# linhthi/BLISS-GNN

Measured on AMD Instinct MI355X. Metric: steps/sec (train step: sample_blocks + gather + SAGE fwd/bwd + Adam + exp3), reddit-like, higher is better.
Workload: dtype bf16

## Files before the change

bliss_gnn_amd/_engine.py:

```python
import contextlib
import ctypes as C
import os

import numpy as np
import torch

from . import _lib
from .graph import Block, Graph

_CHUNK = 1024
_CAP_ERRS = 1 | 2 | 4 | 8 | 64


def _ptr(t):
    return 0 if t is None else t.data_ptr()


def _stream():
    return torch.cuda.current_stream().cuda_stream


def _up8(n):
    return (int(n) + 7) & ~7


class _LayerWs:

    def __init__(self, dev, cap_s, cap_c):
        self.cap_s, self.cap_c = cap_s, cap_c
        self.seg_ptr = torch.empty(cap_s + 1, dtype=torch.int32, device=dev)
        self.seed_acc = torch.empty(60 * cap_s + 64, dtype=torch.uint8, device=dev)
        self.cand_nid = torch.empty(cap_c, dtype=torch.int32, device=dev)
        self.new_id = torch.empty(cap_c, dtype=torch.int32, device=dev)
        self.p = torch.empty(cap_c, dtype=torch.bfloat16, device=dev)
        self.P = torch.empty(cap_c, dtype=torch.bfloat16, device=dev)
        self.uniforms = torch.empty(cap_c, dtype=torch.float32, device=dev)
        self.keys = torch.empty(cap_c, dtype=torch.float32, device=dev)
        self.draw_scr = torch.zeros(int(_lib.lib.bliss_multinomial_draw_scratch_bytes(cap_c)) // 4, dtype=torch.int32, device=dev)
        self.src_cnt = None
        self.tr_temp = None


class DrawState:

    def __init__(self, seed, step, device):
        self.seed = int(seed) & ((1 << 64) - 1)
        self.step_dev = torch.tensor([int(step)], dtype=torch.int64, device=device)

    def step(self):
        return int(self.step_dev.item())


class LayerEngine:

    def __init__(self, g: Graph):
        if g.device.type != "cuda":
            raise RuntimeError("bliss_gnn_amd samples on the GPU only; move the graph with g.to('cuda') "
                               "(the reference's --data-cpu/--use-uva modes are out of scope)")
        self.g = g
        dev = g.device
        V = g.num_nodes()
        self.V, self.Eg = V, g.num_edges()
        if self.Eg >= 2 ** 31:
            raise RuntimeError("int32 edge positions: graphs with >= 2^31 edges are not supported")
        self.scratch_sets = 2
        self._sets = {}
        self.first_pos = torch.full((V,), -1, dtype=torch.int32, device=dev)
        self.acc_p2 = torch.zeros(V, dtype=torch.int64, device=dev)
        self.c_graph = _lib.Graph(g.indptr.data_ptr(), g.indices.data_ptr(), _ptr(g.eid), V, self.Eg)
        self.flags = torch.zeros(16, dtype=torch.int32, device=dev)
        self.fs_ticket = torch.zeros(1, dtype=torch.int32, device=dev)
        self.fuse_scale = os.environ.get("BLISS_FUSE_SCALE", "1") != "0"
        self.flag_err = torch.zeros(1, dtype=torch.int32, device=dev)
        self.n_bins = 0
        for nb in ((int(os.environ["BLISS_NBINS"]),) if os.environ.get("BLISS_NBINS") else (256, 1024)):
            if -(-V // nb) * 12 <= 64 * 1024:
                self.n_bins = nb
                break
        if os.environ.get("BLISS_BINS", "1") == "0" or self.Eg > 2048 * 4096 * 32:
            self.n_bins = 0
        self._bins = None
        self.hist = torch.zeros(32768, dtype=torch.int32, device=dev)
        self.mt_dev = torch.empty(626, dtype=torch.int32, device=dev)
        self.mt_host = torch.empty(626, dtype=torch.int32).pin_memory()
# ... 714 lines not shown
```

bliss_gnn_amd/csrc/common.cuh:

```cuda
#pragma once
#include <hip/hip_runtime.h>
#include <stdint.h>
#include "bliss_gnn.h"

#define BLISS_WAVE 64

#define FRAC_DST 40
#define FRAC_SRC 44
#define FRAC_BLK 36

#define BLISS_ERR_CAP_FRONTIER 1
#define BLISS_ERR_CAP_CAND     2
#define BLISS_ERR_CAP_KEPT     4
#define BLISS_ERR_CAP_EDGES    8
#define BLISS_ERR_NONFINITE   16
#define BLISS_ERR_FIXED_RANGE 32
#define BLISS_ERR_CAP_SEEDS   64
#define BLISS_ERR_RNG_STREAM 128
#define BLISS_ERR_FLAG_TIMEOUT 256

typedef uint16_t bf16_t;

__device__ __forceinline__ float bf2f(bf16_t b) { return __uint_as_float(((uint32_t)b) << 16); }

// ... 52 lines not shown

__device__ __forceinline__ long long bf_to_fixed_wide(bf16_t b, int frac, long long* lo, int* sticky, int* bad) {
  uint32_t e = (b >> 7) & 0xff, m = b & 0x7f;
  if (e == 255) { *bad |= BLISS_ERR_NONFINITE; return 0; }
  if (e == 0) e = 1; else m |= 0x80;
  const int shift = (int)e - 134 + frac;
  const bool neg = (b & 0x8000) != 0;
  if (shift >= 0) {
    if (shift > 55) { *bad |= BLISS_ERR_FIXED_RANGE; return 0; }
    const long long mag = (long long)((uint64_t)m << shift);
    return neg ? -mag : mag;
  }
  const int rs = -shift;
  const uint32_t top = rs >= 8 ? 0u : (m >> rs);
  const uint32_t r = rs >= 8 ? m : (m & ((1u << rs) - 1u));
  if (r) {
    long long l;
    if (rs <= 40) l = (long long)((uint64_t)r << (40 - rs));
    else {
      const int d = rs - 40;
      l = d >= 8 ? 0 : (long long)(r >> d);
      if (d >= 8 || (r & ((1u << d) - 1u))) *sticky = 1;
    }
    *lo += neg ? -l : l;
  }
  return neg ? -(long long)top : (long long)top;
}

__device__ __forceinline__ bf16_t fixed_wide_to_bf(int64_t hi, int64_t lo, int sticky, int frac, int* bad) {
  if (lo == 0 && !sticky) return fixed_to_bf(hi, frac, bad);
  __int128 t = ((__int128)hi << 40) + (__int128)lo;
  if (t == 0) return 0;
  const uint32_t sign = t < 0 ? 0x8000u : 0u;
  const unsigned __int128 mag = t < 0 ? (unsigned __int128)(-t) : (unsigned __int128)t;
  const uint64_t mh = (uint64_t)(mag >> 64), ml = (uint64_t)mag;
  const int msb = mh ? 127 - __clzll((long long)mh) : 63 - __clzll((long long)ml);
  const int f = frac + 40;
  auto round_shift = [&](int sh) -> uint64_t {
    if (sh <= 0) return (uint64_t)(mag << (-sh));
    if (sh > 126) return 0;
    uint64_t q = (uint64_t)(mag >> sh);
    const unsigned __int128 rem = mag & ((((unsigned __int128)1) << sh) - 1), half = ((unsigned __int128)1) << (sh - 1);
    if (rem > half || (rem == half && (sticky || (q & 1)))) q += 1;
    return q;
  };
  if (msb - f + 127 <= 0) return (bf16_t)(sign | (uint32_t)round_shift(f - 133));
  uint64_t q = round_shift(msb - 7);
  int e = msb - f + 127;
  if (q >= 256) { q >>= 1; e += 1; }
  if (e >= 255) { *bad |= BLISS_ERR_FIXED_RANGE; return 0; }
  return (bf16_t)(sign | ((uint32_t)e << 7) | ((uint32_t)q & 0x7f));
}

__device__ __forceinline__ int lane_id() { return threadIdx.x & (BLISS_WAVE - 1); }

__device__ __forceinline__ int64_t shfl_up_i64(int64_t v, int d) {
  int lo = __shfl_up((int)(v & 0xffffffffll), d), hi = __shfl_up((int)(v >> 32), d);
  return ((int64_t)hi << 32) | (uint32_t)lo;
}

template <int CTRL, int ROW_MASK>
__device__ __forceinline__ int dpp_mov0(int v) { return __builtin_amdgcn_update_dpp(0, v, CTRL, ROW_MASK, 0xf, false); }
template <int CTRL, int ROW_MASK>
__device__ __forceinline__ long long dpp_mov0_i64(long long v) {
  const int lo = dpp_mov0<CTRL, ROW_MASK>((int)(v & 0xffffffffll)), hi = dpp_mov0<CTRL, ROW_MASK>((int)(v >> 32));
  return ((long long)hi << 32) | (unsigned)lo;
}
__device__ __forceinline__ int wave_total_i32(int v) {
  v += dpp_mov0<0x111, 0xf>(v); v += dpp_mov0<0x112, 0xf>(v); v += dpp_mov0<0x114, 0xf>(v); v += dpp_mov0<0x118, 0xf>(v);
  v += dpp_mov0<0x142, 0xa>(v); v += dpp_mov0<0x143, 0xc>(v);
  return __builtin_amdgcn_readlane(v, 63);
}
__device__ __forceinline__ int wave_max_u31(int v) {
  v = max(v, dpp_mov0<0x111, 0xf>(v)); v = max(v, dpp_mov0<0x112, 0xf>(v)); v = max(v, dpp_mov0<0x114, 0xf>(v));
  v = max(v, dpp_mov0<0x118, 0xf>(v)); v = max(v, dpp_mov0<0x142, 0xa>(v)); v = max(v, dpp_mov0<0x143, 0xc>(v));
  return __builtin_amdgcn_readlane(v, 63);
}
__device__ __forceinline__ int bf_exp_field(bf16_t b) { const int e = (b >> 7) & 0xff; return e == 0 ? 1 : e; }
__device__ __forceinline__ int rel_frac(int frac, int emax) { const int s = 126 - emax; return frac + (s > 0 ? s : 0); }

__device__ __forceinline__ long long wave_total_i64(long long v) {
  v += dpp_mov0_i64<0x111, 0xf>(v); v += dpp_mov0_i64<0x112, 0xf>(v); v += dpp_mov0_i64<0x114, 0xf>(v);
  v += dpp_mov0_i64<0x118, 0xf>(v); v += dpp_mov0_i64<0x142, 0xa>(v); v += dpp_mov0_i64<0x143, 0xc>(v);
  const int lo = __builtin_amdgcn_readlane((int)(v & 0xffffffffll), 63), hi = __builtin_amdgcn_readlane((int)(v >> 32), 63);
  return ((long long)hi << 32) | (unsigned)lo;
}
__device__ __forceinline__ bool wave_single_key(int key, int* k0) {
  const unsigned long long act = __ballot(key >= 0);
  if (!act) { *k0 = -1; return true; }
  *k0 = __builtin_amdgcn_readlane(key, __ffsll((long long)act) - 1);
  return __ballot(key >= 0 && key != *k0) == 0ull;
}

__device__ __forceinline__ void wave_segsum_atomic_i64(int key, int64_t v, unsigned long long* acc) {
  const int lane = lane_id();
  int k0;
  if (wave_single_key(key, &k0)) {
    if (k0 < 0) return;
    const long long tot = wave_total_i64(key >= 0 ? v : 0);
    if (lane == 0 && tot != 0) atomicAdd(acc + k0, (unsigned long long)tot);
    return;
  }
#pragma unroll
  for (int d = 1; d < BLISS_WAVE; d <<= 1) {
    int64_t vu = shfl_up_i64(v, d);
    int ku = __shfl_up(key, d);
// ... 117 lines not shown
```

bliss_gnn_amd/csrc/sampler.hip:

```cpp
#include "common.cuh"
#include "bliss_gnn.h"
#include "prof.h"
#include "edge_q.cuh"
#include <cstdlib>

#ifndef TPB
#define TPB 256
#endif
#define ITEMS 4
#define CHUNK (TPB * ITEMS)

namespace {

#define SPAN (64 * ITEMS)
#define SEG_ZERO_WGS 8
#define LONG_COL 1024

struct EdgeAt {
  int k;
  int64_t pos;
  int src;
};

__device__ __forceinline__ EdgeAt decode(int base, int E, int S, const int* __restrict__ seg_ptr,
                                         const long long* __restrict__ col_base, const int* __restrict__ indices, int* k_hint) {
  EdgeAt r;
  const int e = base + lane_id();
  r.k = wave_segment(seg_ptr, S, base, k_hint);
  r.pos = 0; r.src = 0;
  if (e < E) {
    r.pos = col_base[r.k] + e;
    r.src = indices[r.pos];
  } else r.k = -1;
  return r;
}

__device__ __forceinline__ int chunk_wave_offset(int wave_total, int* sh4, int* chunk_total) {
  const int wave = threadIdx.x >> 6;
  __syncthreads();
  if (lane_id() == 0) sh4[wave] = wave_total;
  __syncthreads();
  int off = 0, tot = 0;
#pragma unroll
  for (int w = 0; w < TPB / 64; ++w) { const int v = sh4[w]; tot += v; if (w < wave) off += v; }
  *chunk_total = tot;
  return off;
}

__device__ __forceinline__ void seg_scan_body(const int64_t* __restrict__ indptr, const int* __restrict__ seeds,
                                              LayerCounts* cnt, int S_host, const int* __restrict__ S_dev, int cap_s,
                                              unsigned long long* __restrict__ seed_acc, int* __restrict__ seg_ptr,
                                              int* __restrict__ local_id, int num_nodes, int* __restrict__ src_cnt, int cap_k,
                                              int* __restrict__ bin_cursor, int n_bins, long long* __restrict__ col_base,
                                              int* __restrict__ span_seg, long long frontier_cap, int* entry_flag,
                                              int wg, int n_wgs, bool keep_sums, int* sh, int* st_sh, int* hub_count = nullptr) {
  if (entry_flag && wg == 0 && threadIdx.x == 0) __hip_atomic_store(entry_flag, 1, __ATOMIC_RELEASE, __HIP_MEMORY_SCOPE_AGENT);
  __shared__ int sh_long;
  if (hub_count && threadIdx.x == 0) sh_long = 0;
  int S = S_host >= 0 ? S_host : *S_dev;
  int bad = 0;
  if (S > cap_s) { S = cap_s; bad |= BLISS_ERR_CAP_SEEDS; }
  if (wg > 0 || n_wgs == 1) {
    const int nz = n_wgs > 1 ? n_wgs - 1 : 1, bz = n_wgs > 1 ? wg - 1 : 0;
    const int t0 = bz * blockDim.x + threadIdx.x, step = nz * blockDim.x;
    for (int i = (keep_sums ? 2 * cap_s : 0) + t0; i < cap_s * 5; i += step) seed_acc[i] = 0ull;
    if (src_cnt) for (int i = t0; i <= cap_k; i += step) src_cnt[i] = 0;
    if (bin_cursor) for (int i = t0; i <= n_bins; i += step) bin_cursor[i] = 0;
    for (int k = t0; k < S; k += step) { const int s = seeds[k]; if (s >= 0 && s < num_nodes) local_id[s] = k; }
    if (n_wgs > 1) return;
  }
  long long run = 0;
  constexpr int G = 4;
  for (int base0 = 0; base0 < S; base0 += G * (int)blockDim.x) {
    int degs[G];
    long long cols[G];
#pragma unroll
    for (int i = 0; i < G; ++i) {
      const int k = base0 + i * (int)blockDim.x + threadIdx.x;
      degs[i] = 0; cols[i] = 0;
      if (k < S) {
        const int s = seeds[k];
        if (s < 0 || s >= num_nodes) { bad |= BLISS_ERR_CAP_CAND; }
        else {
          cols[i] = indptr[s];
          degs[i] = (int)(indptr[s + 1] - cols[i]);
        }
      }
    }
#pragma unroll
    for (int i = 0; i < G; ++i) {
      const int k = base0 + i * (int)blockDim.x + threadIdx.x;
      if (base0 + i * (int)blockDim.x >= S) break;
      const int deg = degs[i];
      int tot, ex = block_excl_scan(deg, sh, &tot);
      const long long start = run + ex;
      if (k < S) {
        seg_ptr[k] = (int)start;
        col_base[k] = deg > 0 ? cols[i] - start : 0;
      }
      if (hub_count) {
        const bool is_long = k < S && deg > LONG_COL;
        const unsigned long long mask = __ballot(is_long);
        if (mask) {
          int base_l = 0;
          if (lane_id() == 0) base_l = atomicAdd(&sh_long, __popcll(mask));
          base_l = __shfl(base_l, 0);
          if (is_long) hub_count[base_l + __popcll(mask & ((1ull << lane_id()) - 1ull))] = k;
        }
      }
      if (run + tot <= frontier_cap) {
        st_sh[threadIdx.x] = (int)(k < S ? start : run + tot);
        __syncthreads();
        const long long sp_end = (run + tot + SPAN - 1) / SPAN;
        for (long long sp = (run + SPAN - 1) / SPAN + threadIdx.x; sp < sp_end; sp += blockDim.x) {
          const int p = (int)(sp * SPAN);
          int t = 0;
#pragma unroll
          for (int step = 512; step >= 1; step >>= 1) if (st_sh[t + step] <= p) t += step;
          span_seg[sp] = base0 + i * (int)blockDim.x + t;
        }
      }
      run += tot;
      if (run > frontier_cap) bad |= BLISS_ERR_CAP_FRONTIER;
    }
  }
  int any_bad = __syncthreads_or(bad);
  if (threadIdx.x == 0) {
    if (hub_count) hub_count[cap_s] = sh_long;
    seg_ptr[S] = (int)run;
    cnt->S = S; cnt->E = (any_bad & BLISS_ERR_CAP_FRONTIER) ? 0 : (int)run;
    cnt->C = 0; cnt->K = 0; cnt->B = 0; cnt->iters = 0; cnt->all_one = 0; cnt->c = 1.0;
    cnt->err = any_bad;
  }
}

__global__ void __launch_bounds__(1024) k_seg_scan(const int64_t* __restrict__ indptr, const int* __restrict__ seeds,
                                                   LayerCounts* cnt, int S_host, const int* __restrict__ S_dev, int cap_s,
                                                   unsigned long long* __restrict__ seed_acc, int* __restrict__ seg_ptr,
                                                   int* __restrict__ local_id, int num_nodes, int* __restrict__ src_cnt, int cap_k,
                                                   int* __restrict__ bin_cursor, int n_bins, long long* __restrict__ col_base,
                                                   int* __restrict__ span_seg, long long frontier_cap, int* entry_flag,
                                                   int keep_sums, int* hub_count) {
  __shared__ int sh[17];
  __shared__ int st_sh[1024];
  seg_scan_body(indptr, seeds, cnt, S_host, S_dev, cap_s, seed_acc, seg_ptr, local_id, num_nodes, src_cnt, cap_k, bin_cursor, n_bins,
                col_base, span_seg, frontier_cap, entry_flag, blockIdx.x, gridDim.x, keep_sums != 0, sh, st_sh, hub_count);
}

template <bool BANDIT>
__global__ void __launch_bounds__(TPB) k_frontier_pass1(const int64_t* __restrict__ indptr, const int* __restrict__ indices,
                                                        const bf16_t* __restrict__ w, const int* __restrict__ seeds,
                                                        const int* __restrict__ seg_ptr, const long long* __restrict__ col_base,
    const int* __restrict__ span_seg, LayerCounts* cnt,
                                                        const int* __restrict__ local_id, unsigned* first_pos,
                                                        unsigned long long* acc_w) {
  const int S = cnt->S, E = cnt->E;
  const int nspans = (E + SPAN - 1) / SPAN;
  int bad = 0;
  for (int sp = blockIdx.x * (TPB / 64) + (threadIdx.x >> 6); sp < nspans; sp += gridDim.x * (TPB / 64)) {
    int hint = span_seg[sp];
#pragma unroll
    for (int i = 0; i < ITEMS; ++i) {
      const int base = sp * SPAN + i * 64;
      if (base >= E) break;
      const int e = base + lane_id();
      EdgeAt a = decode(base, E, S, seg_ptr, col_base, indices, &hint);
      int64_t term = 0;
      if (a.k >= 0) {
        if (local_id[a.src] < 0) {
          if (__hip_atomic_load(first_pos + a.src, __ATOMIC_RELAXED, __HIP_MEMORY_SCOPE_AGENT) > (unsigned)e)
            atomicMin(first_pos + a.src, (unsigned)e);
        }
        if (BANDIT) term = bf_to_fixed(w[a.pos], FRAC_DST, &bad);
      }
      if (BANDIT) wave_segsum_atomic_i64(a.k, term, acc_w);
    }
  }
  if (bad) atomicOr(&cnt->err, bad);
}

template <bool BANDIT>
__global__ void __launch_bounds__(TPB) k_frontier_pass2(const int64_t* __restrict__ indptr, const int* __restrict__ indices,
                                                        const bf16_t* __restrict__ w, const int* __restrict__ seeds,
                                                        const int* __restrict__ seg_ptr, const long long* __restrict__ col_base,
    const int* __restrict__ span_seg, LayerCounts* cnt,
                                                        const unsigned* __restrict__ first_pos,
                                                        const unsigned long long* __restrict__ acc_w,
                                                        unsigned long long* acc_q, int* __restrict__ chunk_cnt,
                                                        float eta_f, float ome_f) {
  __shared__ int sh4[TPB / 64];
  const int S = cnt->S, E = cnt->E;
  const int nchunks = (E + CHUNK - 1) / CHUNK;
  int bad = 0;
  for (int chunk = blockIdx.x; chunk < nchunks; chunk += gridDim.x) {
    int nfirst = 0, hint = span_seg[chunk * ITEMS + (threadIdx.x >> 6)];
#pragma unroll
    for (int i = 0; i < ITEMS; ++i) {
      const int base = chunk * CHUNK + (threadIdx.x >> 6) * SPAN + i * 64;
      if (base >= E) break;
// ... 114 lines not shown
  __shared__ int lh[HIST_BINS];
  const int S = cnt->S;
  const int C = min(cnt->C, cap_c);
  if ((int)blockIdx.x * FIN_TPB >= C) return;
  {
    int4* lh4 = reinterpret_cast<int4*>(lh);
    for (int b = threadIdx.x; b < HIST_BINS / 4; b += FIN_TPB) lh4[b] = make_int4(0, 0, 0, 0);
  }
  __syncthreads();
  int bad = 0;
  for (int id = blockIdx.x * FIN_TPB + threadIdx.x; id < C; id += gridDim.x * FIN_TPB) {
    int g;
    if (id < S) { g = seeds[id]; cand_nid[id] = g; } else g = cand_nid[id];
    const unsigned long long raw = acc_p2[g];
    acc_p2[g] = 0;
    first_pos[g] = 0xffffffffu;
    bf16_t pj;
    if (uniform_nodes) pj = raw ? (bf16_t)0x3f80 : (bf16_t)0;
    else pj = f2bf(sqrtf(bf2f(fixed_to_bf((int64_t)raw, FRAC_SRC, &bad))));
    p[id] = pj;
    if (pj < HIST_BINS) atomicAdd(&lh[pj], 1); else bad |= BLISS_ERR_NONFINITE;
  }
  __syncthreads();
  {
    const int4* lh4 = reinterpret_cast<const int4*>(lh);
    for (int b = threadIdx.x; b < HIST_BINS / 4; b += FIN_TPB) {
      const int4 v = lh4[b];
      if (v.x | v.y | v.z | v.w) {
        if (v.x) atomicAdd(hist + 4 * b, v.x);
        if (v.y) atomicAdd(hist + 4 * b + 1, v.y);
        if (v.z) atomicAdd(hist + 4 * b + 2, v.z);
        if (v.w) atomicAdd(hist + 4 * b + 3, v.w);
      }
    }
  }
  if (bad) atomicOr(&cnt->err, bad);
}

#define BIN_TPB 1024
#ifndef BIN_ITEMS
#define BIN_ITEMS 4
#endif
#define BIN_BATCH (BIN_TPB * BIN_ITEMS)
#define MAX_BINS 1024
#ifndef COL_TPB
#define COL_TPB 1024
#endif
#ifndef COL_R
#define COL_R 16
#endif
#ifndef COL_RB
#define COL_RB 8
#endif
#define COL_BIG (COL_R * 64)
static_assert(LONG_COL == COL_BIG, "k_seg_scan lists the columns k_col_sums treats as long");
#ifndef BINRED_TPB
#define BINRED_TPB 1024
#endif

template <int NT>
__device__ __forceinline__ int block_max_u31(int v, long long* sh) {
  v = wave_max_u31(v);
  __syncthreads();
  if (lane_id() == 0) sh[threadIdx.x >> 6] = v;
  __syncthreads();
  int t = 0;
#pragma unroll
  for (int w = 0; w < NT / 64; ++w) t = max(t, (int)sh[w]);
  return t;
}

template <int NT>
__device__ __forceinline__ long long block_sum2_i64(long long a, long long b, long long* sh2, long long* b_out) {
  a = wave_total_i64(a);
  b = wave_total_i64(b);
  __syncthreads();
  if (lane_id() == 0) { sh2[threadIdx.x >> 6] = a; sh2[NT / 64 + (threadIdx.x >> 6)] = b; }
  __syncthreads();
  long long ta = 0, tb = 0;
#pragma unroll
  for (int w = 0; w < NT / 64; ++w) { ta += sh2[w]; tb += sh2[NT / 64 + w]; }
  *b_out = tb;
  return ta;
}

template <int NT>
__device__ __forceinline__ long long block_sum_i64(long long v, long long* sh) {
  v = wave_total_i64(v);
  __syncthreads();
  if (lane_id() == 0) sh[threadIdx.x >> 6] = v;
  __syncthreads();
  long long t = 0;
#pragma unroll
  for (int w = 0; w < NT / 64; ++w) t += sh[w];
  return t;
}

__device__ __forceinline__ void col_store(int k, long long ws_fixed, long long qs_fixed, bf16_t wsum, int n, float eta_f,
                                          unsigned long long* acc_w, unsigned long long* acc_q, uint2* seed_coef, int* bad) {
  acc_w[k] = (unsigned long long)ws_fixed; acc_q[k] = (unsigned long long)qs_fixed;
  const bf16_t qsum = fixed_to_bf(qs_fixed, FRAC_DST, bad);
  seed_coef[k] = make_uint2((unsigned)wsum | ((unsigned)qsum << 16), __float_as_uint(rbf((1.0f / (float)n) * eta_f)));
}

__global__ void __launch_bounds__(COL_TPB) k_col_sums(const int64_t* __restrict__ indptr, const bf16_t* __restrict__ w,
                                                      const int* __restrict__ seeds, const int* __restrict__ seg_ptr,
                                                      const long long* __restrict__ col_base, const int* __restrict__ span_seg,
                                                      LayerCounts* cnt, unsigned long long* __restrict__ acc_w,
                                                      unsigned long long* __restrict__ acc_q, float eta_f, float ome_f,
                                                      uint2* __restrict__ seed_coef, int n_wave_wgs,
                                                      const int* __restrict__ long_list, int cap_s) {
  __shared__ long long sh[COL_TPB / 64];
  __shared__ long long sh2[2 * COL_TPB / 64];
  const int S = cnt->S, tid = threadIdx.x, lane = lane_id();
  if (cnt->E == 0) return;
  int bad = 0;
  const int n_block_wgs = (int)gridDim.x - n_wave_wgs;
  if ((int)blockIdx.x < n_wave_wgs)
  for (int k = blockIdx.x * (COL_TPB / 64) + (tid >> 6); k < S; k += n_wave_wgs * (COL_TPB / 64)) {
    const int s0 = seg_ptr[k], n = seg_ptr[k + 1] - s0;
    if (n == 0 || n > COL_BIG) continue;
    const long long p0 = col_base[k] + s0;
    bf16_t wr[COL_R];
    long long part = 0;
    int emax = 1;
#pragma unroll
    for (int r = 0; r < COL_R; ++r) {
      const int i = lane + r * 64;
      wr[r] = 0;
      if (i < n) wr[r] = w[p0 + i];
    }
#pragma unroll
    for (int r = 0; r < COL_R; ++r)
      if (lane + r * 64 < n) emax = max(emax, bf_exp_field(wr[r]));
    const int wfrac = rel_frac(FRAC_DST, wave_max_u31(emax));
    long long part_lo = 0;
    int sticky = 0;
#pragma unroll
    for (int r = 0; r < COL_R; ++r)
      if (lane + r * 64 < n) part += bf_to_fixed_wide(wr[r], wfrac, &part_lo, &sticky, &bad);
    const long long ws_fixed = wave_total_i64(part);
    bf16_t wsum;
    if (__ballot(part_lo != 0 || sticky) == 0ull) wsum = fixed_to_bf(ws_fixed, wfrac, &bad);
    else wsum = fixed_wide_to_bf(ws_fixed, wave_total_i64(part_lo), __ballot(sticky) != 0ull, wfrac, &bad);
    const float a = rbf((1.0f / (float)n) * eta_f);
    part = 0;
#pragma unroll
    for (int r = 0; r < COL_R; ++r) {
      const int i = lane + r * 64;
      if (i < n) part += bf_to_fixed(edge_q_pre(wr[r], wsum, a, ome_f), FRAC_DST, &bad);
    }
    const long long qs_fixed = wave_total_i64(part);
    if (lane == 0) col_store(k, ws_fixed, qs_fixed, wsum, n, eta_f, acc_w, acc_q, seed_coef, &bad);
  }
  if ((int)blockIdx.x >= n_wave_wgs)
  for (int li = (int)blockIdx.x - n_wave_wgs, n_long = long_list[cap_s]; li < n_long; li += n_block_wgs) {
    const int k = long_list[li];
    const int s0 = seg_ptr[k], n = seg_ptr[k + 1] - s0;
    if (n <= COL_BIG) continue;
    const long long p0 = col_base[k] + s0;
    bf16_t wr[COL_RB];
    long long part = 0;
    int emax = 1;
#pragma unroll
    for (int r = 0; r < COL_RB; ++r) {
      const int i = tid + r * COL_TPB;
      wr[r] = 0;
      if (i < n) wr[r] = w[p0 + i];
    }
#pragma unroll
    for (int r = 0; r < COL_RB; ++r)
      if (tid + r * COL_TPB < n) emax = max(emax, bf_exp_field(wr[r]));
#pragma unroll 8
    for (int i = tid + COL_RB * COL_TPB; i < n; i += COL_TPB) emax = max(emax, bf_exp_field(w[p0 + i]));
    const int wfrac = rel_frac(FRAC_DST, block_max_u31<COL_TPB>(emax, sh));
    long long part_lo = 0;
    int sticky = 0;
#pragma unroll
    for (int r = 0; r < COL_RB; ++r)
      if (tid + r * COL_TPB < n) part += bf_to_fixed_wide(wr[r], wfrac, &part_lo, &sticky, &bad);
#pragma unroll 8
    for (int i = tid + COL_RB * COL_TPB; i < n; i += COL_TPB)
      part += bf_to_fixed_wide(w[p0 + i], wfrac, &part_lo, &sticky, &bad);
    long long lost;
    const long long ws_fixed = block_sum2_i64<COL_TPB>(part, (part_lo != 0 || sticky) ? 1 : 0, sh2, &lost);
    bf16_t wsum;
    if (lost == 0) wsum = fixed_to_bf(ws_fixed, wfrac, &bad);
    else {
      const long long lo_tot = block_sum_i64<COL_TPB>(part_lo, sh);
      const long long st_tot = block_sum_i64<COL_TPB>(sticky, sh);
      wsum = fixed_wide_to_bf(ws_fixed, lo_tot, st_tot != 0, wfrac, &bad);
    }
    const float a = rbf((1.0f / (float)n) * eta_f);
    part = 0;
#pragma unroll
    for (int r = 0; r < COL_RB; ++r) {
      const int i = tid + r * COL_TPB;
      if (i < n) part += bf_to_fixed(edge_q_pre(wr[r], wsum, a, ome_f), FRAC_DST, &bad);
    }
#pragma unroll 8
    for (int i = tid + COL_RB * COL_TPB; i < n; i += COL_TPB) part += bf_to_fixed(edge_q_pre(w[p0 + i], wsum, a, ome_f), FRAC_DST, &bad);
    const long long qs_fixed = block_sum_i64<COL_TPB>(part, sh);
    if (tid == 0) col_store(k, ws_fixed, qs_fixed, wsum, n, eta_f, acc_w, acc_q, seed_coef, &bad);
  }
  if (bad) atomicOr(&cnt->err, bad);
}

template <bool BANDIT>
__global__ void __launch_bounds__(BIN_TPB) k_bin_scatter(const int64_t* __restrict__ indptr, const int* __restrict__ indices,
                                                     const bf16_t* __restrict__ w, const int* __restrict__ seeds,
                                                     const int* __restrict__ seg_ptr, const long long* __restrict__ col_base,
    const int* __restrict__ span_seg, LayerCounts* cnt,
                                                     const unsigned long long* __restrict__ acc_w,
                                                     const unsigned long long* __restrict__ acc_q, float eta_f, float ome_f,
                                                     int uniform_nodes, int n_bins, int log2_bins, long long bin_cap, int* bin_cursor,
                                                     unsigned long long* __restrict__ bin_rec, unsigned* __restrict__ bitmap,
                                                     const uint2* __restrict__ seed_coef) {
  __shared__ int hist[MAX_BINS];
  __shared__ int gbase[MAX_BINS];
  const int S = cnt->S, E = cnt->E, tid = threadIdx.x;
  const int nb = (E + BIN_BATCH - 1) / BIN_BATCH;
  const int bmask = n_bins - 1;
  int bad = 0;
  for (int batch = blockIdx.x; batch < nb; batch += gridDim.x) {
    for (int b = tid; b < n_bins; b += BIN_TPB) hist[b] = 0;
    if (tid < BIN_BATCH / 32) bitmap[batch * (BIN_BATCH / 32) + tid] = 0u;
    __syncthreads();
    int srcs[BIN_ITEMS], ranks[BIN_ITEMS];
    bf16_t ts[BIN_ITEMS];
    const int wbase = batch * BIN_BATCH + (tid >> 6) * (64 * BIN_ITEMS);
    int hint = span_seg[wbase >> 8];
#pragma unroll
    for (int j = 0; j < BIN_ITEMS; ++j) {
      ranks[j] = -1; srcs[j] = 0; ts[j] = 0;
      const int base = wbase + j * 64;
      if (base >= E) continue;
      EdgeAt a = decode(base, E, S, seg_ptr, col_base, indices, &hint);
      if (a.k >= 0) {
        bf16_t t;
        if (uniform_nodes) {
          t = (bf16_t)0x3f80;
        } else if (BANDIT) {
          const uint2 cf = seed_coef[a.k];
          bf16_t q = edge_q_pre(w[a.pos], (bf16_t)(cf.x & 0xffffu), __uint_as_float(cf.y), ome_f);
          float r = rbf(bf2f(q) / bf2f((bf16_t)(cf.x >> 16)));
          t = f2bf(r * r);
        } else {
          float x = bf2f(w[a.pos]);
          t = f2bf(x * x);
        }
        srcs[j] = a.src; ts[j] = t;
        ranks[j] = atomicAdd(&hist[a.src & bmask], 1);
      }
    }
    __syncthreads();
    for (int b = tid; b < n_bins; b += BIN_TPB) {
// ... 687 lines not shown

extern "C" {

int bliss_layer_counts_bytes(void) { return (int)sizeof(LayerCounts); }

int bliss_flag_raise(int32_t* flag, void* stream) {
  if (!flag) return BLISS_EINVAL;
  k_flag_raise<<<1, 64, 0, (hipStream_t)stream>>>(flag);
  return (int)hipGetLastError();
}

int bliss_flag_wait(int32_t* flag, int32_t* err_word, void* stream) {
  if (!flag) return BLISS_EINVAL;
  k_flag_wait<<<1, 64, 0, (hipStream_t)stream>>>(flag, err_word, g_flag_spin_bound);
  return (int)hipGetLastError();
}

int bliss_flag_set_spin_bound(int64_t spins) {
  if (spins < 1) return BLISS_EINVAL;
  g_flag_spin_bound = spins;
  return 0;
}

int bliss_frontier_prob(const bliss_graph_t* g, const bliss_node_maps_t* m, const void* w_pos, const int32_t* seeds,
                        int32_t n_seeds, const int32_t* n_seeds_dev, int32_t cap_s, int mode, float eta_f,
                        float one_minus_eta_f, int64_t frontier_bound, const bliss_layer_ws_t* ws, void* stream_) {
  if (!g || !m || !seeds || !ws || !w_pos || cap_s <= 0 || !ws->hist || !ws->span_seg) return BLISS_EINVAL;
  if (n_seeds < 0 && !n_seeds_dev) return BLISS_EINVAL;
  if (n_seeds > cap_s) return BLISS_EINVAL;
  const int uniform_nodes = (mode & BLISS_MODE_UNIFORM_NODES) ? 1 : 0;
  const bool partials_only = (mode & BLISS_MODE_PARTIALS) != 0;
  mode &= ~(BLISS_MODE_UNIFORM_NODES | BLISS_MODE_PARTIALS);
  if (mode != BLISS_MODE_BANDIT && mode != BLISS_MODE_LADIES) return BLISS_EINVAL;
  if (partials_only && ws->n_bins <= 0) return BLISS_EINVAL;
  hipStream_t st = (hipStream_t)stream_;
  LayerCounts* cnt = (LayerCounts*)ws->counts;
  const bf16_t* w = (const bf16_t*)w_pos;
  unsigned long long* acc_w = (unsigned long long*)ws->seed_acc;
  unsigned long long* acc_q = acc_w + cap_s;
  const long long* col_base = (const long long*)(acc_w + 5 * (size_t)cap_s);
  if (frontier_bound < 1) frontier_bound = 1;
  const int ge = grid_for(frontier_bound, TPB), gc = grid_for(frontier_bound, CHUNK);
  const bool binned = ws->n_bins > 0;
  int log2_bins = 0, slots = 0;
  if (binned) {
    while ((1 << log2_bins) < ws->n_bins) ++log2_bins;
    slots = (g->num_nodes + ws->n_bins - 1) >> log2_bins;
    if ((1 << log2_bins) != ws->n_bins || ws->n_bins > MAX_BINS || (size_t)slots * 12 > 64 * 1024 || ws->bin_cap <= 0 ||
        g->num_edges > (long long)MAX_TILES * BTILE * 32 || !ws->bin_cursor || !ws->bin_rec || !ws->bitmap || !ws->word_prefix || !ws->touched_key || !ws->touched_sum)
      return BLISS_EINVAL;
  }
  const long long fcap = (long long)(g->num_edges < 0x7fffffffll ? g->num_edges : 0x7fffffffll);
  const bool col_sums = binned && mode == BLISS_MODE_BANDIT;
  int* long_list = (int*)(acc_w + 7 * (size_t)cap_s);
  PROF_LAUNCH(BK_SEG_SCAN, st, k_seg_scan<<<1 + SEG_ZERO_WGS, 1024, 0, st>>>(g->indptr, seeds, cnt, n_seeds, n_seeds_dev, cap_s, acc_w, ws->seg_ptr,
                                                            m->local_id, g->num_nodes, ws->src_cnt, ws->cap_k,
                                                            binned ? ws->bin_cursor : nullptr, ws->n_bins, (long long*)col_base, ws->span_seg,
                                                            fcap, ws->entry_flag, col_sums ? 1 : 0, col_sums ? long_list : nullptr));
  if (binned) {
    unsigned long long* seed_p2 = acc_w + 4 * (size_t)cap_s;
    uint2* seed_coef = (uint2*)(acc_w + 6 * (size_t)cap_s);
    unsigned long long* bin_rec = (unsigned long long*)ws->bin_rec;
    const int gb = grid_for(frontier_bound, BIN_BATCH);
    const int n_wave_wgs = grid_for(cap_s, COL_TPB / 64, 2048);
    if (col_sums)
      PROF_LAUNCH(BK_COL_SUMS, st, k_col_sums<<<n_wave_wgs + (cap_s < 2048 ? cap_s : 2048), COL_TPB, 0, st>>>(g->indptr, w, seeds, ws->seg_ptr, col_base, ws->span_seg, cnt, acc_w, acc_q, eta_f, one_minus_eta_f, seed_coef, n_wave_wgs, long_list, cap_s));
    if (mode == BLISS_MODE_BANDIT)
      PROF_LAUNCH(BK_BIN_SCATTER, st, k_bin_scatter<true><<<gb, BIN_TPB, 0, st>>>(g->indptr, g->indices, w, seeds, ws->seg_ptr, col_base, ws->span_seg, cnt, acc_w, acc_q, eta_f, one_minus_eta_f, uniform_nodes, ws->n_bins, log2_bins, ws->bin_cap, ws->bin_cursor, bin_rec, ws->bitmap, seed_coef));
    else
      PROF_LAUNCH(BK_BIN_SCATTER, st, k_bin_scatter<false><<<gb, BIN_TPB, 0, st>>>(g->indptr, g->indices, w, seeds, ws->seg_ptr, col_base, ws->span_seg, cnt, acc_w, acc_q, eta_f, one_minus_eta_f, uniform_nodes, ws->n_bins, log2_bins, ws->bin_cap, ws->bin_cursor, bin_rec, ws->bitmap, seed_coef));
    PROF_LAUNCH(BK_BIN_REDUCE, st, k_bin_reduce<<<ws->n_bins, BINRED_TPB, (size_t)slots * 12, st>>>(
        cnt, ws->n_bins, log2_bins, ws->bin_cap, ws->bin_cursor, bin_rec, g->num_nodes, slots, m->local_id, seed_p2,
        (unsigned long long*)ws->touched_key, (unsigned long long*)ws->touched_sum, ws->bitmap, ws->cap_c));
    if (partials_only) return (int)hipGetLastError();
    int* tile_sum = ws->word_prefix;
    int* word_prefix = ws->word_prefix + MAX_TILES;
    PROF_LAUNCH(BK_BITMAP_SCAN, st, k_bitmap_tiles<<<grid_for(frontier_bound, (int64_t)BTILE * 32, MAX_TILES), 1024, 0, st>>>(ws->bitmap, word_prefix, tile_sum, cnt));
    int gf = (ws->cap_c + FIN_TPB - 1) / FIN_TPB;
    if (gf < 1) gf = 1;
    if (gf > 512) gf = 512;
    PROF_LAUNCH(BK_CAND_NUMBER, st, k_cand_number<<<gf, FIN_TPB, 0, st>>>(
        seeds, cnt, ws->cand_nid, m->local_id, seed_p2, (const unsigned long long*)ws->touched_key,
        (const unsigned long long*)ws->touched_sum, ws->bitmap, word_prefix, tile_sum, (bf16_t*)ws->p, ws->hist, ws->cap_c, uniform_nodes,
        FusedScale{ws->fs_ticket, ws->fs_fanout, ws->fs_eps, ws->fs_rng_ctl, ws->fs_layer_off, ws->fs_is_last, ws->fs_rng_cap, ws->chunk_cnt}));
    return (int)hipGetLastError();
  }
  if (mode == BLISS_MODE_BANDIT) {
    PROF_LAUNCH(BK_PASS1, st, k_frontier_pass1<true><<<ge, TPB, 0, st>>>(g->indptr, g->indices, w, seeds, ws->seg_ptr, col_base, ws->span_seg, cnt, m->local_id, m->first_pos, acc_w));
    PROF_LAUNCH(BK_PASS2, st, k_frontier_pass2<true><<<gc, TPB, 0, st>>>(g->indptr, g->indices, w, seeds, ws->seg_ptr, col_base, ws->span_seg, cnt, m->first_pos, acc_w, acc_q, ws->chunk_cnt, eta_f, one_minus_eta_f));
  } else {
    PROF_LAUNCH(BK_PASS1, st, k_frontier_pass1<false><<<ge, TPB, 0, st>>>(g->indptr, g->indices, w, seeds, ws->seg_ptr, col_base, ws->span_seg, cnt, m->local_id, m->first_pos, acc_w));
    PROF_LAUNCH(BK_PASS2, st, k_frontier_pass2<false><<<gc, TPB, 0, st>>>(g->indptr, g->indices, w, seeds, ws->seg_ptr, col_base, ws->span_seg, cnt, m->first_pos, acc_w, acc_q, ws->chunk_cnt, eta_f, one_minus_eta_f));
  }
  PROF_LAUNCH(BK_CHUNK_SCAN, st, k_chunk_scan<<<1, 1024, 0, st>>>(ws->chunk_cnt, cnt, 0, ws->cap_c));
  if (mode == BLISS_MODE_BANDIT)
    PROF_LAUNCH(BK_PASS3, st, k_frontier_pass3<true><<<gc, TPB, 0, st>>>(g->indptr, g->indices, w, seeds, ws->seg_ptr, col_base, ws->span_seg, cnt, m->first_pos, acc_w, acc_q, ws->chunk_cnt, m->local_id, ws->cand_nid, (unsigned long long*)m->acc_p2, eta_f, one_minus_eta_f, ws->cap_c, uniform_nodes));
  else
    PROF_LAUNCH(BK_PASS3, st, k_frontier_pass3<false><<<gc, TPB, 0, st>>>(g->indptr, g->indices, w, seeds, ws->seg_ptr, col_base, ws->span_seg, cnt, m->first_pos, acc_w, acc_q, ws->chunk_cnt, m->local_id, ws->cand_nid, (unsigned long long*)m->acc_p2, eta_f, one_minus_eta_f, ws->cap_c, uniform_nodes));
  {
    int gf = (ws->cap_c + FIN_TPB * 8 - 1) / (FIN_TPB * 8);
    if (gf < 1) gf = 1;
    if (gf > 256) gf = 256;
    PROF_LAUNCH(BK_CAND_FINALIZE, st, k_cand_finalize<<<gf, FIN_TPB, 0, st>>>(
        seeds, cnt, ws->cand_nid, (unsigned long long*)m->acc_p2, m->first_pos, (bf16_t*)ws->p, ws->hist, ws->cap_c, uniform_nodes));
  }
  return (int)hipGetLastError();
}

int bliss_poisson_select(const bliss_layer_ws_t* ws, int32_t fanout, double eps, const float* uniforms,
                         int32_t* uniforms_offset_dev, int32_t* rng_ctl, int is_last, int32_t rng_cap_total,
                         int64_t cand_bound, void* stream_) {
  if (!ws || !uniforms || fanout < 0 || (rng_ctl && !uniforms_offset_dev)) return BLISS_EINVAL;
  hipStream_t st = (hipStream_t)stream_;
  LayerCounts* cnt = (LayerCounts*)ws->counts;
  if (cand_bound < 1) cand_bound = 1;
  if (cand_bound > ws->cap_c) cand_bound = ws->cap_c;
  if (!ws->fs_ticket)
    PROF_LAUNCH(BK_POISSON_SCALE, st, k_poisson_scale<<<1, 1024, 0, st>>>(ws->hist, cnt, fanout, eps, rng_ctl, uniforms_offset_dev, is_last, rng_cap_total, ws->chunk_cnt));
  PROF_LAUNCH(BK_SELECT2, st, k_select_fused<<<grid_for(cand_bound, CHUNK, 1 << 20), TPB, 0, st>>>(
// ... 87 lines not shown
```

Measured before the change: 1459.

## Add fast-path bf16-to-fixed conversion and reorder long-column work in col sums

Adds a cheap bf16-to-fixed conversion for values whose exponents fall in a range where the sum is exact, and falls back to the wide/sticky path only when a wave or block detects an out-of-range value. The seg scan now records long columns as (k, n, p0) entries, putting very long columns first and the rest from the end, so column-sum blocks start on the heaviest hubs and avoid re-reading seg_ptr and col_base. Register use is cut by packing bf16 values in pairs, using scalar base pointers, and one wave per column indexing without a loop. The block-workgroup count is capped and launch bounds are added to raise occupancy. The fallback path re-reads the column, which costs extra memory traffic when odd values occur.

```diff
diff --git a/bliss_gnn_amd/_engine.py b/bliss_gnn_amd/_engine.py
--- a/bliss_gnn_amd/_engine.py
+++ b/bliss_gnn_amd/_engine.py
@@ -29,7 +29,7 @@
     def __init__(self, dev, cap_s, cap_c):
         self.cap_s, self.cap_c = cap_s, cap_c
         self.seg_ptr = torch.empty(cap_s + 1, dtype=torch.int32, device=dev)
-        self.seed_acc = torch.empty(60 * cap_s + 64, dtype=torch.uint8, device=dev)
+        self.seed_acc = torch.empty(72 * cap_s + 64, dtype=torch.uint8, device=dev)
         self.cand_nid = torch.empty(cap_c, dtype=torch.int32, device=dev)
         self.new_id = torch.empty(cap_c, dtype=torch.int32, device=dev)
         self.p = torch.empty(cap_c, dtype=torch.bfloat16, device=dev)
diff --git a/bliss_gnn_amd/csrc/common.cuh b/bliss_gnn_amd/csrc/common.cuh
--- a/bliss_gnn_amd/csrc/common.cuh
+++ b/bliss_gnn_amd/csrc/common.cuh
@@ -128,6 +128,23 @@
   return (bf16_t)(sign | ((uint32_t)e << 7) | ((uint32_t)q & 0x7f));
 }
 
+struct PlainRange { unsigned lo, span; };
+__device__ __forceinline__ PlainRange bf_plain_range(int frac) {
+  int e_lo = 134 - frac, e_hi = 189 - frac;
+  if (e_hi > 254) e_hi = 254;
+  PlainRange r;
+  r.lo = e_lo <= 1 ? 0u : (unsigned)e_lo << 7;
+  const unsigned end = e_hi < 1 ? 0u : (unsigned)(e_hi + 1) << 7;
+  r.span = end > r.lo ? end - r.lo : 0u;
+  return r;
+}
+__device__ __forceinline__ bool bf_is_plain(bf16_t b, PlainRange r) { return (unsigned)b - r.lo < r.span; }
+__device__ __forceinline__ long long bf_fixed_plain(bf16_t b, int frac) {
+  const unsigned ef = (unsigned)b >> 7, m = (b & 0x7fu) | (ef ? 0x80u : 0u);
+  const int shift = (int)(ef ? ef : 1u) - 134 + frac;
+  return (long long)((uint64_t)m << (shift & 63));
+}
+
 __device__ __forceinline__ int lane_id() { return threadIdx.x & (BLISS_WAVE - 1); }
 
 __device__ __forceinline__ int64_t shfl_up_i64(int64_t v, int d) {
diff --git a/bliss_gnn_amd/csrc/sampler.hip b/bliss_gnn_amd/csrc/sampler.hip
--- a/bliss_gnn_amd/csrc/sampler.hip
+++ b/bliss_gnn_amd/csrc/sampler.hip
@@ -15,6 +15,12 @@
 #define SPAN (64 * ITEMS)
 #define SEG_ZERO_WGS 8
 #define LONG_COL 1024
+#define LONG_FIRST 4096
+
+struct alignas(8) ColEnt {
+  int k, n;
+  long long p0;
+};
 
 struct EdgeAt {
   int k;
@@ -53,10 +59,10 @@
                                               int* __restrict__ local_id, int num_nodes, int* __restrict__ src_cnt, int cap_k,
                                               int* __restrict__ bin_cursor, int n_bins, long long* __restrict__ col_base,
                                               int* __restrict__ span_seg, long long frontier_cap, int* entry_flag,
-                                              int wg, int n_wgs, bool keep_sums, int* sh, int* st_sh, int* hub_count = nullptr) {
+                                              int wg, int n_wgs, bool keep_sums, int* sh, int* st_sh, ColEnt* long_list = nullptr) {
   if (entry_flag && wg == 0 && threadIdx.x == 0) __hip_atomic_store(entry_flag, 1, __ATOMIC_RELEASE, __HIP_MEMORY_SCOPE_AGENT);
-  __shared__ int sh_long;
-  if (hub_count && threadIdx.x == 0) sh_long = 0;
+  __shared__ int sh_long[2];
+  if (long_list && threadIdx.x < 2) sh_long[threadIdx.x] = 0;
   int S = S_host >= 0 ? S_host : *S_dev;
   int bad = 0;
   if (S > cap_s) { S = cap_s; bad |= BLISS_ERR_CAP_SEEDS; }
@@ -98,14 +104,22 @@
         seg_ptr[k] = (int)start;
         col_base[k] = deg > 0 ? cols[i] - start : 0;
       }
-      if (hub_count) {
-        const bool is_long = k < S && deg > LONG_COL;
-        const unsigned long long mask = __ballot(is_long);
-        if (mask) {
-          int base_l = 0;
-          if (lane_id() == 0) base_l = atomicAdd(&sh_long, __popcll(mask));
-          base_l = __shfl(base_l, 0);
-          if (is_long) hub_count[base_l + __popcll(mask & ((1ull << lane_id()) - 1ull))] = k;
+      if (long_list) {
+        const bool is_long = k < S && deg > LONG_COL, is_first = is_long && deg > LONG_FIRST;
+        const unsigned long long m_first = __ballot(is_first), m_rest = __ballot(is_long && !is_first);
+        if (m_first | m_rest) {
+          int b_first = 0, b_rest = 0;
+          if (lane_id() == 0) {
+            if (m_first) b_first = atomicAdd(&sh_long[0], __popcll(m_first));
+            if (m_rest) b_rest = atomicAdd(&sh_long[1], __popcll(m_rest));
+          }
+          b_first = __shfl(b_first, 0); b_rest = __shfl(b_rest, 0);
+          if (is_long) {
+            const unsigned long long below = (1ull << lane_id()) - 1ull;
+            const int slot = is_first ? b_first + __popcll(m_first & below) : cap_s - 1 - (b_rest + __popcll(m_rest & below));
+            ColEnt ent; ent.k = k; ent.n = deg; ent.p0 = cols[i];
+            long_list[slot] = ent;
+          }
         }
       }
       if (run + tot <= frontier_cap) {
@@ -126,7 +140,7 @@
   }
   int any_bad = __syncthreads_or(bad);
   if (threadIdx.x == 0) {
-    if (hub_count) hub_count[cap_s] = sh_long;
+    if (long_list) { int* n_long = (int*)(long_list + cap_s); n_long[0] = sh_long[0]; n_long[1] = sh_long[1]; }
     seg_ptr[S] = (int)run;
     cnt->S = S; cnt->E = (any_bad & BLISS_ERR_CAP_FRONTIER) ? 0 : (int)run;
     cnt->C = 0; cnt->K = 0; cnt->B = 0; cnt->iters = 0; cnt->all_one = 0; cnt->c = 1.0;
@@ -140,11 +154,11 @@
                                                    int* __restrict__ local_id, int num_nodes, int* __restrict__ src_cnt, int cap_k,
                                                    int* __restrict__ bin_cursor, int n_bins, long long* __restrict__ col_base,
                                                    int* __restrict__ span_seg, long long frontier_cap, int* entry_flag,
-                                                   int keep_sums, int* hub_count) {
+                                                   int keep_sums, ColEnt* long_list) {
   __shared__ int sh[17];
   __shared__ int st_sh[1024];
   seg_scan_body(indptr, seeds, cnt, S_host, S_dev, cap_s, seed_acc, seg_ptr, local_id, num_nodes, src_cnt, cap_k, bin_cursor, n_bins,
-                col_base, span_seg, frontier_cap, entry_flag, blockIdx.x, gridDim.x, keep_sums != 0, sh, st_sh, hub_count);
+                col_base, span_seg, frontier_cap, entry_flag, blockIdx.x, gridDim.x, keep_sums != 0, sh, st_sh, long_list);
 }
 
 template <bool BANDIT>
@@ -365,6 +379,9 @@
 #ifndef COL_RB
 #define COL_RB 8
 #endif
+#ifndef COL_BLOCK_WGS
+#define COL_BLOCK_WGS 512
+#endif
 #define COL_BIG (COL_R * 64)
 static_assert(LONG_COL == COL_BIG, "k_seg_scan lists the columns k_col_sums treats as long");
 #ifndef BINRED_TPB
@@ -409,6 +426,19 @@
   return t;
 }
 
+template <int N>
+struct PackedBf {
+  unsigned v[N / 2];
+  __device__ __forceinline__ void set(int r, bf16_t x) { v[r >> 1] = (r & 1) ? (v[r >> 1] | ((unsigned)x << 16)) : (unsigned)x; }
+  __device__ __forceinline__ bf16_t get(int r) const { return (bf16_t)((r & 1) ? v[r >> 1] >> 16 : v[r >> 1] & 0xffffu); }
+};
+
+__device__ __forceinline__ const bf16_t* uniform_ptr(const bf16_t* p) {
+  const unsigned long long v = (unsigned long long)p;
+  const unsigned lo = __builtin_amdgcn_readfirstlane((int)(unsigned)v), hi = __builtin_amdgcn_readfirstlane((int)(unsigned)(v >> 32));
+  return (const bf16_t*)(((unsigned long long)hi << 32) | lo);
+}
+
 __device__ __forceinline__ void col_store(int k, long long ws_fixed, long long qs_fixed, bf16_t wsum, int n, float eta_f,
                                           unsigned long long* acc_w, unsigned long long* acc_q, uint2* seed_coef, int* bad) {
   acc_w[k] = (unsigned long long)ws_fixed; acc_q[k] = (unsigned long long)qs_fixed;
@@ -416,105 +446,174 @@
   seed_coef[k] = make_uint2((unsigned)wsum | ((unsigned)qsum << 16), __float_as_uint(rbf((1.0f / (float)n) * eta_f)));
 }
 
-__global__ void __launch_bounds__(COL_TPB) k_col_sums(const int64_t* __restrict__ indptr, const bf16_t* __restrict__ w,
+__global__ void __launch_bounds__(COL_TPB, 8) k_col_sums(const int64_t* __restrict__ indptr, const bf16_t* __restrict__ w,
                                                       const int* __restrict__ seeds, const int* __restrict__ seg_ptr,
                                                       const long long* __restrict__ col_base, const int* __restrict__ span_seg,
                                                       LayerCounts* cnt, unsigned long long* __restrict__ acc_w,
                                                       unsigned long long* __restrict__ acc_q, float eta_f, float ome_f,
-                                                      uint2* __restrict__ seed_coef, int n_wave_wgs,
-                                                      const int* __restrict__ long_list, int cap_s) {
+                                                      uint2* __restrict__ seed_coef, int n_block_wgs,
+                                                      const ColEnt* __restrict__ long_list, int cap_s) {
   __shared__ long long sh[COL_TPB / 64];
   __shared__ long long sh2[2 * COL_TPB / 64];
-  const int S = cnt->S, tid = threadIdx.x, lane = lane_id();
-  if (cnt->E == 0) return;
+  const int tid = threadIdx.x, lane = lane_id();
+  const int* n_long = (const int*)(long_list + cap_s);
+  const int S = cnt->S, E = cnt->E, n_first = n_long[0], n_all = n_first + n_long[1];
+  if (E == 0) return;
   int bad = 0;
-  const int n_block_wgs = (int)gridDim.x - n_wave_wgs;
-  if ((int)blockIdx.x < n_wave_wgs)
-  for (int k = blockIdx.x * (COL_TPB / 64) + (tid >> 6); k < S; k += n_wave_wgs * (COL_TPB / 64)) {
-    const int s0 = seg_ptr[k], n = seg_ptr[k + 1] - s0;
-    if (n == 0 || n > COL_BIG) continue;
-    const long long p0 = col_base[k] + s0;
-    bf16_t wr[COL_R];
+  const int bid_wave = (int)blockIdx.x, bid_block = (int)blockIdx.x - ((int)gridDim.x - n_block_wgs);
+  if (bid_block < 0) {
+  const int k = bid_wave * (COL_TPB / 64) + __builtin_amdgcn_readfirstlane(tid >> 6);
+  const int s0 = k < S ? seg_ptr[k] : 0, n = k < S ? seg_ptr[k + 1] - s0 : 0;
+  const long long cb = k < S ? col_base[k] : 0;
+  if (n > 0 && n <= COL_BIG) {
+    const bf16_t* wc = uniform_ptr(w + (cb + s0));
+    PackedBf<COL_R> wr;
     long long part = 0;
     int emax = 1;
-#pragma unroll
-    for (int r = 0; r < COL_R; ++r) {
-      const int i = lane + r * 64;
-      wr[r] = 0;
-      if (i < n) wr[r] = w[p0 + i];
+    {
+      bf16_t x[COL_R];
+#pragma unroll
+      for (int r = 0; r < COL_R; ++r) {
+        const int i = lane + r * 64;
+        x[r] = 0;
+        if (i < n) x[r] = wc[i];
+      }
+#pragma unroll
+      for (int r = 0; r < COL_R; ++r) wr.set(r, x[r]);
     }
 #pragma unroll
     for (int r = 0; r < COL_R; ++r)
-      if (lane + r * 64 < n) emax = max(emax, bf_exp_field(wr[r]));
+      if (lane + r * 64 < n) emax = max(emax, bf_exp_field(wr.get(r)));
     const int wfrac = rel_frac(FRAC_DST, wave_max_u31(emax));
-    long long part_lo = 0;
-    int sticky = 0;
+    const PlainRange wr_ok = bf_plain_range(wfrac);
+    bool odd = false;
 #pragma unroll
     for (int r = 0; r < COL_R; ++r)
-      if (lane + r * 64 < n) part += bf_to_fixed_wide(wr[r], wfrac, &part_lo, &sticky, &bad);
-    const long long ws_fixed = wave_total_i64(part);
+      if (r * 64 < n) {
+        odd |= lane + r * 64 < n && !bf_is_plain(wr.get(r), wr_ok);
+        part += bf_fixed_plain(wr.get(r), wfrac);
+      }
+    long long ws_fixed;
     bf16_t wsum;
-    if (__ballot(part_lo != 0 || sticky) == 0ull) wsum = fixed_to_bf(ws_fixed, wfrac, &bad);
-    else wsum = fixed_wide_to_bf(ws_fixed, wave_total_i64(part_lo), __ballot(sticky) != 0ull, wfrac, &bad);
+    if (__ballot(odd) == 0ull) {
+      ws_fixed = wave_total_i64(part);
+      wsum = fixed_to_bf(ws_fixed, wfrac, &bad);
+    } else {
+      long long part_lo = 0;
+      int sticky = 0;
+      part = 0;
+#pragma unroll 4
+      for (int i = lane; i < n; i += 64) part += bf_to_fixed_wide(wc[i], wfrac, &part_lo, &sticky, &bad);
+      ws_fixed = wave_total_i64(part);
+      if (__ballot(part_lo != 0 || sticky) == 0ull) wsum = fixed_to_bf(ws_fixed, wfrac, &bad);
+      else wsum = fixed_wide_to_bf(ws_fixed, wave_total_i64(part_lo), __ballot(sticky) != 0ull, wfrac, &bad);
+    }
     const float a = rbf((1.0f / (float)n) * eta_f);
-    part = 0;
-#pragma unroll
-    for (int r = 0; r < COL_R; ++r) {
-      const int i = lane + r * 64;
-      if (i < n) part += bf_to_fixed(edge_q_pre(wr[r], wsum, a, ome_f), FRAC_DST, &bad);
+    const PlainRange q_ok = bf_plain_range(FRAC_DST);
+    part = 0; odd = false;
+#pragma unroll
+    for (int r = 0; r < COL_R; ++r)
+      if (r * 64 < n) {
+        const bool in = lane + r * 64 < n;
+        const bf16_t q = edge_q_pre(wr.get(r), wsum, a, ome_f);
+        odd |= in && !bf_is_plain(q, q_ok);
+        part += in ? bf_fixed_plain(q, FRAC_DST) : 0ll;
+      }
+    if (__ballot(odd) != 0ull) {
+      part = 0;
+#pragma unroll 4
+      for (int i = lane; i < n; i += 64) part += bf_to_fixed(edge_q_pre(wc[i], wsum, a, ome_f), FRAC_DST, &bad);
     }
     const long long qs_fixed = wave_total_i64(part);
     if (lane == 0) col_store(k, ws_fixed, qs_fixed, wsum, n, eta_f, acc_w, acc_q, seed_coef, &bad);
   }
-  if ((int)blockIdx.x >= n_wave_wgs)
-  for (int li = (int)blockIdx.x - n_wave_wgs, n_long = long_list[cap_s]; li < n_long; li += n_block_wgs) {
-    const int k = long_list[li];
-    const int s0 = seg_ptr[k], n = seg_ptr[k + 1] - s0;
-    if (n <= COL_BIG) continue;
-    const long long p0 = col_base[k] + s0;
-    bf16_t wr[COL_RB];
+  }
+  if (bid_block >= 0) {
+  for (int li = bid_block; li < n_all; li += n_block_wgs) {
+    const ColEnt ent = long_list[li < n_first ? li : cap_s - 1 - (li - n_first)];
+    const int k = ent.k, n = ent.n;
+    const bf16_t* wc = uniform_ptr(w + ent.p0);
+    int t = tid;
+    asm volatile("" : "+v"(t));
+    const int wave0 = __builtin_amdgcn_readfirstlane(t & ~63);
+    PackedBf<COL_RB> wr;
     long long part = 0;
     int emax = 1;
-#pragma unroll
-    for (int r = 0; r < COL_RB; ++r) {
-      const int i = tid + r * COL_TPB;
-      wr[r] = 0;
-      if (i < n) wr[r] = w[p0 + i];
+    {
+      bf16_t x[COL_RB];
+#pragma unroll
+      for (int r = 0; r < COL_RB; ++r) {
+        const int i = t + r * COL_TPB;
+        x[r] = 0;
+        if (i < n) x[r] = wc[i];
+      }
+#pragma unroll
+      for (int r = 0; r < COL_RB; ++r) wr.set(r, x[r]);
     }
 #pragma unroll
     for (int r = 0; r < COL_RB; ++r)
-      if (tid + r * COL_TPB < n) emax = max(emax, bf_exp_field(wr[r]));
+      if (t + r * COL_TPB < n) emax = max(emax, bf_exp_field(wr.get(r)));
 #pragma unroll 8
-    for (int i = tid + COL_RB * COL_TPB; i < n; i += COL_TPB) emax = max(emax, bf_exp_field(w[p0 + i]));
+    for (int i = t + COL_RB * COL_TPB; i < n; i += COL_TPB) emax = max(emax, bf_exp_field(wc[i]));
     const int wfrac = rel_frac(FRAC_DST, block_max_u31<COL_TPB>(emax, sh));
-    long long part_lo = 0;
-    int sticky = 0;
+    const PlainRange wr_ok = bf_plain_range(wfrac);
+    bool odd = false;
 #pragma unroll
     for (int r = 0; r < COL_RB; ++r)
-      if (tid + r * COL_TPB < n) part += bf_to_fixed_wide(wr[r], wfrac, &part_lo, &sticky, &bad);
+      if (wave0 + r * COL_TPB < n) {
+        odd |= t + r * COL_TPB < n && !bf_is_plain(wr.get(r), wr_ok);
+        part += bf_fixed_plain(wr.get(r), wfrac);
+      }
 #pragma unroll 8
-    for (int i = tid + COL_RB * COL_TPB; i < n; i += COL_TPB)
-      part += bf_to_fixed_wide(w[p0 + i], wfrac, &part_lo, &sticky, &bad);
+    for (int i = t + COL_RB * COL_TPB; i < n; i += COL_TPB) {
+      const bf16_t b = wc[i];
+      odd |= !bf_is_plain(b, wr_ok);
+      part += bf_fixed_plain(b, wfrac);
+    }
     long long lost;
-    const long long ws_fixed = block_sum2_i64<COL_TPB>(part, (part_lo != 0 || sticky) ? 1 : 0, sh2, &lost);
+    long long ws_fixed = block_sum2_i64<COL_TPB>(part, odd ? 1 : 0, sh2, &lost);
     bf16_t wsum;
     if (lost == 0) wsum = fixed_to_bf(ws_fixed, wfrac, &bad);
     else {
-      const long long lo_tot = block_sum_i64<COL_TPB>(part_lo, sh);
-      const long long st_tot = block_sum_i64<COL_TPB>(sticky, sh);
-      wsum = fixed_wide_to_bf(ws_fixed, lo_tot, st_tot != 0, wfrac, &bad);
+      long long part_lo = 0;
+      int sticky = 0;
+      part = 0;
+#pragma unroll 4
+      for (int i = t; i < n; i += COL_TPB) part += bf_to_fixed_wide(wc[i], wfrac, &part_lo, &sticky, &bad);
+      ws_fixed = block_sum2_i64<COL_TPB>(part, (part_lo != 0 || sticky) ? 1 : 0, sh2, &lost);
+      if (lost == 0) wsum = fixed_to_bf(ws_fixed, wfrac, &bad);
+      else {
+        const long long lo_tot = block_sum_i64<COL_TPB>(part_lo, sh);
+        const long long st_tot = block_sum_i64<COL_TPB>(sticky, sh);
+        wsum = fixed_wide_to_bf(ws_fixed, lo_tot, st_tot != 0, wfrac, &bad);
+      }
     }
     const float a = rbf((1.0f / (float)n) * eta_f);
-    part = 0;
-#pragma unroll
-    for (int r = 0; r < COL_RB; ++r) {
-      const int i = tid + r * COL_TPB;
-      if (i < n) part += bf_to_fixed(edge_q_pre(wr[r], wsum, a, ome_f), FRAC_DST, &bad);
-    }
+    const PlainRange q_ok = bf_plain_range(FRAC_DST);
+    part = 0; odd = false;
+#pragma unroll
+    for (int r = 0; r < COL_RB; ++r)
+      if (wave0 + r * COL_TPB < n) {
+        const bool in = t + r * COL_TPB < n;
+        const bf16_t q = edge_q_pre(wr.get(r), wsum, a, ome_f);
+        odd |= in && !bf_is_plain(q, q_ok);
+        part += in ? bf_fixed_plain(q, FRAC_DST) : 0ll;
+      }
 #pragma unroll 8
-    for (int i = tid + COL_RB * COL_TPB; i < n; i += COL_TPB) part += bf_to_fixed(edge_q_pre(w[p0 + i], wsum, a, ome_f), FRAC_DST, &bad);
-    const long long qs_fixed = block_sum_i64<COL_TPB>(part, sh);
-    if (tid == 0) col_store(k, ws_fixed, qs_fixed, wsum, n, eta_f, acc_w, acc_q, seed_coef, &bad);
+    for (int i = t + COL_RB * COL_TPB; i < n; i += COL_TPB) {
+      const bf16_t q = edge_q_pre(wc[i], wsum, a, ome_f);
+      odd |= !bf_is_plain(q, q_ok);
+      part += bf_fixed_plain(q, FRAC_DST);
+    }
+    long long qs_fixed = block_sum2_i64<COL_TPB>(part, odd ? 1 : 0, sh2, &lost);
+    if (lost != 0) {
+      part = 0;
+#pragma unroll 4
+      for (int i = t; i < n; i += COL_TPB) part += bf_to_fixed(edge_q_pre(wc[i], wsum, a, ome_f), FRAC_DST, &bad);
+      qs_fixed = block_sum_i64<COL_TPB>(part, sh);
+    }
+    if (t == 0) col_store(k, ws_fixed, qs_fixed, wsum, n, eta_f, acc_w, acc_q, seed_coef, &bad);
+  }
   }
   if (bad) atomicOr(&cnt->err, bad);
 }
@@ -1308,7 +1407,7 @@
   }
   const long long fcap = (long long)(g->num_edges < 0x7fffffffll ? g->num_edges : 0x7fffffffll);
   const bool col_sums = binned && mode == BLISS_MODE_BANDIT;
-  int* long_list = (int*)(acc_w + 7 * (size_t)cap_s);
+  ColEnt* long_list = (ColEnt*)(acc_w + 7 * (size_t)cap_s);
   PROF_LAUNCH(BK_SEG_SCAN, st, k_seg_scan<<<1 + SEG_ZERO_WGS, 1024, 0, st>>>(g->indptr, seeds, cnt, n_seeds, n_seeds_dev, cap_s, acc_w, ws->seg_ptr,
                                                             m->local_id, g->num_nodes, ws->src_cnt, ws->cap_k,
                                                             binned ? ws->bin_cursor : nullptr, ws->n_bins, (long long*)col_base, ws->span_seg,
@@ -1318,9 +1417,9 @@
     uint2* seed_coef = (uint2*)(acc_w + 6 * (size_t)cap_s);
     unsigned long long* bin_rec = (unsigned long long*)ws->bin_rec;
     const int gb = grid_for(frontier_bound, BIN_BATCH);
-    const int n_wave_wgs = grid_for(cap_s, COL_TPB / 64, 2048);
+    const int n_wave_wgs = (cap_s + COL_TPB / 64 - 1) / (COL_TPB / 64), n_block_wgs = cap_s < COL_BLOCK_WGS ? cap_s : COL_BLOCK_WGS;
     if (col_sums)
-      PROF_LAUNCH(BK_COL_SUMS, st, k_col_sums<<<n_wave_wgs + (cap_s < 2048 ? cap_s : 2048), COL_TPB, 0, st>>>(g->indptr, w, seeds, ws->seg_ptr, col_base, ws->span_seg, cnt, acc_w, acc_q, eta_f, one_minus_eta_f, seed_coef, n_wave_wgs, long_list, cap_s));
+      PROF_LAUNCH(BK_COL_SUMS, st, k_col_sums<<<n_block_wgs + n_wave_wgs, COL_TPB, 0, st>>>(g->indptr, w, seeds, ws->seg_ptr, col_base, ws->span_seg, cnt, acc_w, acc_q, eta_f, one_minus_eta_f, seed_coef, n_block_wgs, long_list, cap_s));
     if (mode == BLISS_MODE_BANDIT)
       PROF_LAUNCH(BK_BIN_SCATTER, st, k_bin_scatter<true><<<gb, BIN_TPB, 0, st>>>(g->indptr, g->indices, w, seeds, ws->seg_ptr, col_base, ws->span_seg, cnt, acc_w, acc_q, eta_f, one_minus_eta_f, uniform_nodes, ws->n_bins, log2_bins, ws->bin_cap, ws->bin_cursor, bin_rec, ws->bitmap, seed_coef));
     else
```

Measured after the change: 1486 (median of 6 runs). 1.8% higher.
